# MarvelMathesh/sincformer-metacog-speech-enhancement

Hardware: AMD Instinct MI355X
Metric: audio frames/sec/GPU (16 kHz, 512-frame utts) + mask RMSE vs CPU ref (higher is better)
Workload: dtype fp16 MFMA operands (PerceptionAgent, fusion, Conformer GEMMs, heads) + bf16 attention core, fp32 accumulate (ops.POLICIES['mixed']); 1 GPU; B256 x 512-frame utterances (L40880, T512) forward; batch_per_gpu=256, samples=40880, frames_per_utt=512, launch=eager launches, streams=2, precision_policy=mixed

## Files before the change

### include/sincformer_hip.h

```cpp
#ifndef SINCFORMER_HIP_H
#define SINCFORMER_HIP_H
#ifdef __cplusplus
extern "C" {
#endif

#define SFM_OK 0
#define SFM_ERR_ARG (-1)
#define SFM_ERR_SHAPE (-2)
#define SFM_ERR_LAUNCH (-3)
#define SFM_DT_BF16 0
#define SFM_DT_F16 1

#define SFM_EPI_NONE 0
#define SFM_EPI_SWISH 1
#define SFM_EPI_GELU 2
#define SFM_EPI_RESID 3
#define SFM_EPI_GLU 4
#define SFM_EPI_SIGMOID 5
#define SFM_EPI_TANH_SCALE 6
#define SFM_EPI_SIGMA 7
#define SFM_EPI_CPEA 8

int sfm_abi_version(void);

// ... 145 lines not shown
int sfm_sinc_wgrad(const float* x, const void* dy, int dy_f32, float* dfilt, float* scratch, int B, int L, int C, int K,
                   int dtype, void* stream);
long long sfm_sinc_shift_len(int L);
int sfm_sinc_shift_pack(const float* x, void* xs, int B, int L, int dtype, void* stream);
int sfm_sinc_wgrad16(const void* dy, const void* xs, float* dW, int B, int L, int C, int dtype, float* ws, long long ws_floats,
                     void* stream);
int sfm_gn_bwd_reduce(const void* dout, int dout_f32, const void* x1, int x1_f32, const float* sc1, const float* sh1,
                      const float* mean1, const float* rstd1, const void* x2, int x2_f32, const float* sc2,
                      const float* sh2, const float* mean2, const float* rstd2, float* S, int B, int L, int C, int G,
                      int act, int dtype, float* ws, void* stream);
long long sfm_gn_bwd_reduce_ws_floats(int B, int L, int C);
int sfm_gn_bwd_coefs(float* S, const float* gamma1, const float* rstd1, const float* gamma2, const float* rstd2,
                     float* coef1, float* coef2, float* dparam, int B, int L, int C, int G, void* stream);
int sfm_gn_bwd_apply(const void* dout, int dout_f32, const void* x1, int x1_f32, const float* sc1, const float* sh1,
                     const float* mean1, const float* rstd1, const float* coef1, void* dx1, int dx1_f32, const void* x2,
                     int x2_f32, const float* sc2, const float* sh2, const float* mean2, const float* rstd2,
                     const float* coef2, void* dx2, int dx2_f32, int B, int L, int C, int G, int act, int dtype,
                     void* stream);
int sfm_maa_update_stats(const float* sigma, long long n, double* acc, float* stats, long long* num_updates, float momentum,
                         void* stream);
int sfm_maa_forward(const float* sigma, const float* stats, const float* params, float* logits, float* probs,
                    long long* decisions, float* confidence, long long n, void* stream);
int sfm_maa_backward(const float* sigma, const float* stats, const float* params, const float* g_logits, const float* g_probs,
                     const float* g_conf, float* dsigma, void* H1, void* H2, void* dZ1, void* dZ2, void* GL, void* XN,
                     long long n, int dtype, void* stream);
int sfm_vq_forward(const float* x, const float* centroids, int M, float* q, long long* idx, double* acc, long long n,
                   void* stream);
int sfm_vq_backward(const float* x, const long long* idx, const float* centroids, int M, const float* g_q,
                    const float* g_loss, float beta, float* dx, float* dcent, long long n, void* stream);
int sfm_sumsq(const float* g, long long n, double* out, double* ws, void* stream);
int sfm_adamw_step(float* p, float* g, float* m, float* v, long long n, double* ctl, float lr, float beta1, float beta2,
                   float eps, float wd, float inv_scale, float max_norm, int write_back_grad, void* stream);
int sfm_adamw_step_masked(float* p, float* g, float* m, float* v, long long n, double* ctl, float lr, float beta1, float beta2,
                          float eps, float wd, float inv_scale, float max_norm, int write_back_grad, const long long* spans,
                          const float* touched, int n_params, void* stream);
int sfm_adamw_step_scaled(float* p, float* g, float* m, float* v, long long n, double* ctl, float lr, float beta1, float beta2,
                          float eps, float wd, float inv_world, float max_norm, int write_back_grad, const long long* spans,
                          const float* touched, int n_params, float* loss_scale, float growth_factor, float backoff_factor,
                          int growth_interval, void* stream);
long long sfm_tn_ws_floats(int M, int N, int K);
int sfm_gemm16_tn(const void* G, const void* X, float* dW, float* db, int M, int N, int K, int ldg, int ldx, int ldw,
                  int dtype, float* ws, long long ws_floats, void* stream);
int sfm_conv_wgrad16(const void* G, const void* x, float* dW, float* db, int B, int Lout, int Lin, int Cin, int N, int ksize,
                     int stride, int pad, long long x_batch_stride, int ldg, int ldw, int dtype, float* ws, long long ws_floats,
                     void* stream);
long long sfm_colsum_ws_floats(int M, int N);
int sfm_colsum(const void* G, float* out, int M, int N, int ldg, int g_f32, int dtype, float* ws, void* stream);
long long sfm_layernorm_bwd_ws_floats(int M, int D);
int sfm_layernorm_bwd(const float* x, const float* gamma, const float* dy, const float* dres, float* dx,
                      float* dgamma, float* dbeta, int M, int D, int ldx, int ld, float eps, float* ws, void* stream);
int sfm_layernorm_bwd_ex(const float* x, const float* gamma, const void* dy, int dy_16, const float* dres, float* dx,
                         float* dgamma, float* dbeta, int M, int D, int ldx, int ldy, int ld, float eps, int dtype,
                         float* ws, void* stream);
int sfm_layernorm_bwd_next(const float* x, const float* gamma, const void* dy, int dy_16, const float* dres, float* dx,
                           float* dgamma, float* dbeta, int M, int D, int ldx, int ldy, int ld, float eps, int dtype,
                           void* next16, float next_alpha, float next_p, unsigned int next_seed, float* ws, void* stream);
int sfm_ew_train(const void* z, const void* g, void* out, long long M, int N, int mode, int g_f32, int out_f32,
                 float alpha, float p, unsigned int seed, int dtype, void* stream);
long long sfm_col_stats_ws_floats(int M, int C);
int sfm_col_stats(const float* y, const float* aux, const float* mean, const float* rstd, float* S, int M, int C, float* ws,
                  void* stream);
int sfm_add_cols(const float* a, const float* b, float* out, long long M, int C, int Cb, long long lda, long long ldb, long long ldo,
                 void* stream);
int sfm_lstm_hprev16(const float* h, void* out, int B, int T, int H, int dtype, void* stream);
int sfm_bn_finalize(const float* S, const float* gamma, const float* beta, float* run_mean, float* run_var, float* mean,
                    float* rstd, float* sc, float* sh, int C, long long M, float eps, float momentum, int eval_mode,
                    void* stream);
int sfm_bn_swish_bwd(const void* g, const float* y, const float* mean, const float* rstd, const float* gamma,
                     const float* beta, float* S, float* dy, int M, int C, int g_f32, int pass, int dtype,
                     float* ws, void* stream);
long long sfm_dwconv_wgrad_scratch_floats(int B, int T, int C, int KS);
int sfm_dwconv_wgrad(const void* x, const float* dy, float* dw, float* db, float* scratch, int B, int T, int C, int KS,
                     int dtype, void* stream);
int sfm_attention_fwd_train(const void* qkv, void* out, float* lse, int B, int T, int H, int hd, int ldqkv,
                            int ldo, int koff, int voff, long long qkv_batch_stride, long long o_batch_stride,
                            float scale, float p_drop, unsigned int seed, int dtype, void* stream);
int sfm_attention_bwd(const void* qkv, const void* O, const void* dO, const float* lse, float* delta, void* dqkv,
                      int B, int T, int H, int hd, int ldqkv, int ldo, int koff, int voff, float p_drop,
                      unsigned int seed, int dtype, void* stream);
int sfm_lin256(const void* A, const void* W, const float* bias, void* out, int M, int NW, int lda, int ldo, int glu, int dtype,
               int out_dtype, void* stream);
int sfm_ln_lin256(const float* X32, int ldx, const float* lnw, const float* lnb, float eps, const void* W, const float* bias,
                  void* out, int M, int NW, int ldo, int glu, int dtype, int out_dtype, void* stream);
int sfm_headpool_frames_per_tile(int Tin, int Tout);
int sfm_headpool(const void* xd, const void* W, const float* bias, void* pooled, float* gn_partial, int B, int Tin, int Tout, int NW,
                 int lda, int ldp, int gcols, int dtype, void* stream);

int sfm_bilstm_layer(const float* xg, const float* whh, float* out, int B, int T, int H, int dtype, void* stream);
int sfm_bilstm_layer_ex(const float* xg, const float* whh, float* out, int B, int T, int H, int w16, void* stream);
int sfm_bilstm_layer_train_ex(const float* xg, const float* whh, float* out, float* save, int B, int T, int H, int w16, void* stream);
int sfm_bilstm_layer_train(const float* xg, const float* whh, float* out, float* save, int B, int T, int H, int dtype,
                           void* stream);
int sfm_bilstm_layer_bwd(const float* save, const float* whh, const float* dout, float* dxg, int B, int T, int H,
                         void* stream);
int sfm_memory_fwd(const float* emb, const float* params, float* bias_out, float* gate_out, int* top_idx,
                   float* sim_out, int B, int key_dim, int value_dim, int slots, float temperature, void* stream);
long long sfm_memory_param_floats(int key_dim, int value_dim, int slots);
int sfm_memory_bwd(const float* emb, const float* params, const float* d_out, const float* d_gate, float* d_emb,
                   float* dparams, int B, int key_dim, int value_dim, int slots, float temperature, float* ws, void* stream);

#ifdef __cplusplus
}
#endif
#endif
```

### sincformer_metacog_speech_enhancement_amd/functional.py

```python
import math
import numpy as np
import torch

from . import ops

N_FFT, HOP, WIN = 256, 80, 160
N_FREQ = N_FFT // 2 + 1
SINC_ON_16BIT_MFMA = True
FUSE_LD = 1088


def _f32(t):
    return t.detach().float().contiguous()


def sub(sd, prefix):
    p = prefix + "."
    return {k[len(p):]: v for k, v in sd.items() if k.startswith(p)}


def add_to16(x32, y32, C):
    M = x32.numel() // C
    dev = x32.device
    one = _const(dev, C, 1.0)
# ... 259 lines not shown
        bsh = _f32(sd["batch_norm.bias"]) - _f32(sd["batch_norm.running_mean"]) * bsc + _f32(sd["depthwise.bias"]) * bsc
        folded = (_f32(sd["depthwise.weight"].reshape(D, KS)).t().contiguous(), bsc.contiguous(), bsh.contiguous())
    return {"dw_folded": folded, "ln_w": _f32(sd["layer_norm.weight"]), "ln_b": _f32(sd["layer_norm.bias"]),
            "pw1": ops.pack_linear(sd["pointwise1.weight"].reshape(2 * D, D), sd["pointwise1.bias"], glu=True),
            "dw_w": _f32(sd["depthwise.weight"].reshape(D, -1)), "dw_b": _f32(sd["depthwise.bias"]),
            "bn_w": _f32(sd["batch_norm.weight"]), "bn_b": _f32(sd["batch_norm.bias"]),
            "bn_m": _f32(sd["batch_norm.running_mean"]), "bn_v": _f32(sd["batch_norm.running_var"]),
            "pw2": ops.pack_linear(sd["pointwise2.weight"].reshape(D, D), sd["pointwise2.bias"])}


def pack_block(sd, num_heads=4, index=None):
    with ops.stage("block", index):
        return {"ff1": pack_ffn(sub(sd, "ff1")), "mhsa": pack_mhsa(sub(sd, "mhsa"), num_heads), "conv": pack_convmod(sub(sd, "conv")),
                "ff2": pack_ffn(sub(sd, "ff2")), "fn_w": _f32(sd["final_norm.weight"]), "fn_b": _f32(sd["final_norm.bias"]),
                "index": index}


def _ln16(x32, w, b, act=0):
    out = torch.empty(x32.shape, device=x32.device, dtype=ops.compute_dtype())
    ops.layernorm(x32, w, b, out16=out, act=act)
    return out


def _ffn_fusable(x32, pk):
    return FUSED_FFN and "fused" in pk and x32.is_contiguous()


def ffn_forward_ln(x32, pk, ln_w, ln_b, ln_f32, want_y):
    w1, b1, w2, b2 = pk["fused"]
    return ops.ffn_fused_ln(x32, pk["ln_w"], pk["ln_b"], w1, b1, w2, b2, ln_w, ln_b, ln_f32, want_y=want_y, alpha=0.5)


def ffn_forward(x32, pk):
    if FUSED_FFN and "fused" in pk and x32.is_contiguous():
        w1, b1, w2, b2 = pk["fused"]
        return ops.ffn_fused(x32, pk["ln_w"], pk["ln_b"], w1, b1, w2, b2, alpha=0.5)
    h = _ln16(x32, pk["ln_w"], pk["ln_b"])
    u = ops.linear16(h, pk["w1"], epi=ops.EPI_SWISH)
    return ops.linear16(u, pk["w2"], epi=ops.EPI_RESID, resid=x32, alpha=0.5)


def mhsa_forward(x32, pk, B, T, H, h=None, index=None, seg=None):
    D = x32.shape[1]
    bdt = ops.compute_dtype()
    adt = ops.stage_dtype("attn", index) if D // H == 64 else bdt
    if pk["heads"] != H:
        raise RuntimeError("packed attention weights were scaled for %d heads, got %d" % (pk["heads"], H))
    if h is None:
        qkv = ops.ln_linear16(x32, pk["ln_w"], pk["ln_b"], pk["win"], out_dtype=adt)
    else:
        qkv = ops.linear16(h, pk["win"], out_dtype=adt)
    if seg is not None:
        tb = seg.tables(x32.device, H if D // H == 64 else None)
        args = (qkv, tb["frame_off"], tb["attn_items", H] if D // H == 64 else None, seg.B, seg.max_T, seg.sum_T, H, D // H)
        if adt is bdt:
            o = ops.attention_varlen(*args, prescaled=True, sum_T2=seg.sum_T2)
        else:
            with ops.stage("attn", index):
                o = ops.attention_varlen(*args, prescaled=True, out_dtype=bdt, sum_T2=seg.sum_T2)
    elif adt is bdt:
        o = ops.attention(qkv, B, T, H, D // H, prescaled=True)
    else:
        with ops.stage("attn", index):
            o = ops.attention(qkv, B, T, H, D // H, prescaled=True, out_dtype=bdt)
    return ops.linear16(o, pk["wout"], epi=ops.EPI_RESID, resid=x32, alpha=1.0)


def _dw_folded_any(pk):
    f = pk["dw_folded"] or pk.get("dw_folded_any")
    if f is None:
        bsc = pk["bn_w"] * torch.rsqrt(pk["bn_v"] + 1e-5)
        bsh = pk["bn_b"] - pk["bn_m"] * bsc + pk["dw_b"] * bsc
        f = pk["dw_folded_any"] = (pk["dw_w"].t().contiguous(), bsc.contiguous(), bsh.contiguous())
    return f


def convmod_forward(x32, pk, B, T, seg=None):
    D = x32.shape[1]
    g = ops.ln_linear16(x32, pk["ln_w"], pk["ln_b"], pk["pw1"], epi=ops.EPI_GLU)
    if seg is not None:
        tb = seg.tables(x32.device)
        wT, sc, sh = _dw_folded_any(pk)
        d = ops.dwconv_folded_varlen(g, wT, sc, sh, tb["frame_off"], tb["conv_tiles"], seg.B, seg.max_T, seg.sum_T, D)
    elif pk["dw_folded"] is not None:
        d = ops.dwconv_folded(g, pk["dw_folded"][0], pk["dw_folded"][1], pk["dw_folded"][2], B, T, D)
    else:
        d = ops.dwconv_bn_swish(g, pk["dw_w"], pk["dw_b"], pk["bn_w"], pk["bn_b"], pk["bn_m"], pk["bn_v"], B, T, D)
    return ops.linear16(d, pk["pw2"], epi=ops.EPI_RESID, resid=x32, alpha=1.0)


def block_forward(x32, pk, B, T, H, want16=False, seg=None):
    with ops.stage("block", pk.get("index")):
        return _block_forward(x32, pk, B, T, H, want16, seg)


def _block_forward(x32, pk, B, T, H, want16, seg=None):
    if _ffn_fusable(x32, pk["ff1"]) and x32.shape[1] == 256:
        x, h = ffn_forward_ln(x32, pk["ff1"], pk["mhsa"]["ln_w"], pk["mhsa"]["ln_b"], False, True)
        x = mhsa_forward(x, pk["mhsa"], B, T, H, h=h, index=pk.get("index"), seg=seg)
        x = convmod_forward(x, pk["conv"], B, T, seg=seg)
        if not want16 and _ffn_fusable(x, pk["ff2"]):
            return ffn_forward_ln(x, pk["ff2"], pk["fn_w"], pk["fn_b"], True, False)[1]
        x = ffn_forward(x, pk["ff2"])
    else:
        x = ffn_forward(x32, pk["ff1"])
        x = mhsa_forward(x, pk["mhsa"], B, T, H, index=pk.get("index"), seg=seg)
        x = convmod_forward(x, pk["conv"], B, T, seg=seg)
        x = ffn_forward(x, pk["ff2"])
    out = torch.empty_like(x)
    out16 = torch.empty(x.shape, device=x.device, dtype=ops.compute_dtype()) if want16 else None
    ops.layernorm(x, pk["fn_w"], pk["fn_b"], out16=out16, out32=out)
    return (out, out16) if want16 else out


def pack_complex_conformer(sd, num_blocks, num_heads=4):
    nf2 = sd["input_proj.weight"].shape[1]
    with ops.stage("front"):
        win = ops.pack_linear(sd["input_proj.weight"], sd["input_proj.bias"], k_pad_to=ops.round_up(nf2, 64))
    with ops.stage("tail"):
        wout = ops.pack_linear(sd["output_proj.weight"], sd["output_proj.bias"])
    return {"in": win, "out": wout,
            "blocks": [pack_block(sub(sd, "blocks.%d" % i), num_heads, i) for i in range(num_blocks)], "nf2": nf2}


def complex_conformer_core(x16, pk, B, T, H, out_dtype=None):
    with ops.stage("front"):
        x = ops.linear16(x16, pk["in"], out_dtype=torch.float32)
    skip = x
    for bp in pk["blocks"]:
        x = block_forward(x, bp, B, T, H)
    with ops.stage("tail"):
        y16 = add_to16(x, skip, x.shape[1])
        return ops.linear16(y16, pk["out"], out_dtype=out_dtype or ops.compute_dtype())


def complex_conformer_forward(stft_real, stft_imag, pk, H):
    B, T, nf = stft_real.shape
    M = B * T
    sr, si = stft_real.contiguous(), stft_imag.contiguous()
    ld = pk["in"].Kpad
    with ops.stage("front"):
        x16 = torch.empty(M, ld, device=sr.device, dtype=ops.compute_dtype())
        ops.convert_rows(sr, x16, M, nf, nf, nf, ld)
        ops.convert_rows(si, x16[:, nf:], M, nf, ld - nf, nf, ld)
    y = complex_conformer_core(x16, pk, B, T, H, out_dtype=torch.float32).reshape(B, T, 2 * nf)
    return y[..., :nf], y[..., nf:]


def pack_perception(sd, sample_rate):
    with ops.stage("pa"):
        return _pack_perception(sd, sample_rate)


def _pack_perception(sd, sample_rate):
    pk = {"fs": float(sample_rate)}
    for k in ("low_hz_", "band_hz_", "window", "n_"):
        pk[k] = _f32(sd["sinc_conv." + k]).reshape(-1)
    pk["K"] = pk["window"].numel()
    pk["C0"] = pk["low_hz_"].numel()
    pk["sn_w"], pk["sn_b"] = _f32(sd["sinc_norm.weight"]), _f32(sd["sinc_norm.bias"])
    pk["blocks"] = []
    for i in range(3):
        s = sub(sd, "conv_blocks.%d" % i)
        cout = s["main.0.weight"].shape[0]
        pk["blocks"].append({
            "c1": ops.pack_linear(s["main.0.weight"], s["main.0.bias"]), "g1w": _f32(s["main.1.weight"]), "g1b": _f32(s["main.1.bias"]),
# ... 350 lines not shown
```

### sincformer_metacog_speech_enhancement_amd/lib.py

```python
import ctypes
import os

import torch

_HERE = os.path.dirname(os.path.abspath(__file__))
LIB_PATH = os.environ.get("SFM_LIB_PATH") or os.path.join(_HERE, "libsincformer_hip.so")

c_vp = ctypes.c_void_p
c_i = ctypes.c_int
c_ll = ctypes.c_longlong
c_f = ctypes.c_float

SIGNATURES = {
    "sfm_abi_version": [],
    "sfm_gemm16": [c_vp, c_vp, c_vp, c_vp, c_vp, c_vp, c_i, c_i, c_i, c_i, c_i, c_i, c_i, c_i, c_ll, c_i, c_i, c_i,
                   c_i, c_ll, c_i, c_ll, c_f, c_i, c_i, c_i, c_i, c_i, c_vp],
    "sfm_gemm16_ex": [c_vp, c_vp, c_vp, c_vp, c_vp, c_vp, c_i, c_i, c_i, c_i, c_i, c_i, c_i, c_i, c_ll, c_i, c_i, c_i,
                   c_i, c_ll, c_i, c_ll, c_f, c_i, c_i, c_i, c_i, c_i, c_i, c_vp],
    "sfm_gemm16_train": [c_vp, c_vp, c_vp, c_vp, c_vp, c_vp, c_i, c_i, c_i, c_i, c_i, c_i, c_i, c_i, c_ll, c_i, c_i, c_i,
                   c_i, c_ll, c_i, c_ll, c_f, c_i, c_i, c_i, c_i, c_i, c_i, c_f, ctypes.c_uint, c_vp],
    "sfm_conv16p": [c_vp, c_vp, c_vp, c_vp, c_vp, c_vp, c_vp, c_vp, c_vp, c_vp, c_vp, c_vp, c_vp, c_vp, c_i, c_i, c_i, c_i, c_i,
                    c_i, c_i, c_i, c_i, c_i, c_vp],
    "sfm_framed_gemm_f32": [c_vp, c_vp, c_vp, c_vp, c_vp, c_vp, c_i, c_i, c_i, c_ll, c_i, c_i, c_i, c_i, c_i, c_i,
                            c_i, c_ll, c_ll, c_ll, c_i, c_i, c_i, c_i, c_vp],
# ... 14 lines not shown
    "sfm_pool_time_affine": [c_vp, c_vp, c_vp, c_vp, c_vp, c_i, c_i, c_i, c_i, c_ll, c_ll, c_i, c_vp],
    "sfm_pool_time_affine16": [c_vp, c_i, c_vp, c_vp, c_vp, c_vp, c_i, c_i, c_i, c_i, c_ll, c_ll, c_i, c_vp],
    "sfm_stft_lognorm_pack": [c_vp, c_vp, c_vp, c_ll, c_i, c_i, c_ll, c_i, c_vp],
    "sfm_stft_lognorm_bwd": [c_vp, c_vp, c_vp, c_vp, c_vp, c_ll, c_i, c_ll, c_vp],
    "sfm_polar_mask": [c_vp, c_vp, c_vp, c_vp, c_vp, c_vp, c_vp, c_vp, c_vp, c_vp, c_i, c_ll, c_i, c_f, c_ll, c_ll,
                       c_vp],
    "sfm_complex_mul": [c_vp, c_vp, c_vp, c_vp, c_vp, c_vp, c_ll, c_vp],
    "sfm_istft_ola": [c_vp, c_vp, c_vp, c_i, c_i, c_i, c_i, c_i, c_i, c_ll, c_vp],
    "sfm_pack_spec": [c_vp, c_vp, c_vp, c_ll, c_i, c_i, c_ll, c_vp],
    "sfm_sinc_filters": [c_vp, c_vp, c_vp, c_vp, c_vp, c_vp, c_i, c_i, c_i, c_f, c_f, c_f, c_vp],
    "sfm_ffn_fused": [c_vp, c_vp, c_vp, c_vp, c_vp, c_vp, c_vp, c_vp, c_i, c_i, c_i, c_f, c_f, c_i, c_vp],
    "sfm_ffn_fused_ln": [c_vp, c_vp, c_vp, c_vp, c_vp, c_vp, c_vp, c_vp, c_i, c_i, c_i, c_f, c_f, c_vp, c_vp, c_vp, c_i, c_i,
                         c_vp],
    "sfm_sinc_fir16_tiles": [c_i],
    "sfm_sinc_fir16": [c_vp, c_vp, c_vp, c_vp, c_vp, c_i, c_i, c_i, c_i, c_i, c_i, c_vp],
    "sfm_sinc_fir16_ex": [c_vp, c_vp, c_vp, c_vp, c_vp, c_i, c_i, c_i, c_i, c_i, c_i, c_i, c_vp],
    "sfm_framed_gemm_split16": [c_vp, c_vp, c_vp, c_vp, c_vp, c_i, c_i, c_i, c_ll, c_i, c_i, c_i, c_i, c_i, c_i, c_i, c_i, c_ll,
                                c_ll, c_i, c_vp],
    "sfm_wave_moments": [c_vp, c_vp, c_vp, c_i, c_i, c_vp, c_vp],
    "sfm_spec_sums": [c_vp, c_vp, c_vp, c_vp, c_vp, c_ll, c_vp, c_vp],
    "sfm_enhancer_loss_finalize": [c_vp, c_vp, c_vp, c_vp, c_i, c_i, c_ll, c_i, c_vp, c_vp],
    "sfm_sisnr_bwd": [c_vp, c_vp, c_vp, c_vp, c_i, c_i, c_f, c_vp],
    "sfm_spec_loss_bwd": [c_vp, c_vp, c_vp, c_vp, c_vp, c_vp, c_vp, c_ll, c_i, c_ll, c_i, c_i, c_f, c_vp],
    "sfm_stft_adjoint_ola": [c_vp, c_vp, c_vp, c_i, c_i, c_i, c_i, c_i, c_i, c_i, c_vp],
    "sfm_polar_mask_bwd": [c_vp, c_vp, c_vp, c_vp, c_vp, c_vp, c_vp, c_vp, c_ll, c_ll, c_i, c_f, c_ll, c_ll, c_vp],
    "sfm_attention_bwd_generic": [c_vp, c_vp, c_vp, c_vp, c_vp, c_vp, c_i, c_i, c_i, c_i, c_i, c_i, c_i, c_i, c_f, ctypes.c_uint, c_i,
                                  c_vp],
    "sfm_ssnr_frames": [c_vp, c_vp, c_vp, c_i, c_i, c_i, c_i, c_f, c_f, c_vp],
    "sfm_stoi_frames": [c_vp, c_vp, c_vp, c_vp, c_vp, c_vp, c_vp, c_i, c_i, c_i, c_vp],
    "sfm_lsd_frames": [c_vp, c_vp, c_vp, c_vp, c_vp, c_i, c_i, c_i, c_vp],
    "sfm_ssnr_frames_varlen": [c_vp, c_vp, c_vp, c_vp, c_vp, c_i, c_i, c_i, c_i, c_f, c_f, c_vp],
    "sfm_stoi_frames_varlen": [c_vp, c_vp, c_vp, c_vp, c_vp, c_vp, c_vp, c_vp, c_i, c_i, c_i, c_vp],
    "sfm_lsd_frames_varlen": [c_vp, c_vp, c_vp, c_vp, c_vp, c_vp, c_i, c_i, c_i, c_vp],
    "sfm_wave_moments_varlen": [c_vp, c_vp, c_vp, c_vp, c_i, c_i, c_vp],
    "sfm_sinc_wgrad_scratch_floats": [c_i, c_i, c_i, c_i],
    "sfm_sinc_wgrad": [c_vp, c_vp, c_i, c_vp, c_vp, c_i, c_i, c_i, c_i, c_i, c_vp],
    "sfm_sinc_shift_len": [c_i],
    "sfm_sinc_shift_pack": [c_vp, c_vp, c_i, c_i, c_i, c_vp],
    "sfm_sinc_wgrad16": [c_vp, c_vp, c_vp, c_i, c_i, c_i, c_i, c_vp, c_ll, c_vp],
    "sfm_gemm16_swish": [c_vp, c_vp, c_vp, c_vp, c_vp, c_vp, c_i, c_i, c_i, c_i, c_i, c_i, c_i, c_i, c_f, ctypes.c_uint, c_i, c_vp],
    "sfm_gn_bwd_reduce": [c_vp, c_i, c_vp, c_i, c_vp, c_vp, c_vp, c_vp, c_vp, c_i, c_vp, c_vp, c_vp, c_vp, c_vp, c_i, c_i, c_i,
                          c_i, c_i, c_i, c_vp, c_vp],
    "sfm_gn_bwd_coefs": [c_vp, c_vp, c_vp, c_vp, c_vp, c_vp, c_vp, c_vp, c_i, c_i, c_i, c_i, c_vp],
    "sfm_gn_bwd_apply": [c_vp, c_i, c_vp, c_i, c_vp, c_vp, c_vp, c_vp, c_vp, c_vp, c_i, c_vp, c_i, c_vp, c_vp, c_vp, c_vp,
                         c_vp, c_vp, c_i, c_i, c_i, c_i, c_i, c_i, c_i, c_vp],
    "sfm_maa_update_stats": [c_vp, c_ll, c_vp, c_vp, c_vp, c_f, c_vp],
    "sfm_maa_forward": [c_vp, c_vp, c_vp, c_vp, c_vp, c_vp, c_vp, c_ll, c_vp],
    "sfm_maa_backward": [c_vp, c_vp, c_vp, c_vp, c_vp, c_vp, c_vp, c_vp, c_vp, c_vp, c_vp, c_vp, c_vp, c_ll, c_i, c_vp],
    "sfm_vq_forward": [c_vp, c_vp, c_i, c_vp, c_vp, c_vp, c_ll, c_vp],
    "sfm_vq_backward": [c_vp, c_vp, c_vp, c_i, c_vp, c_vp, c_f, c_vp, c_vp, c_ll, c_vp],
    "sfm_sumsq": [c_vp, c_ll, c_vp, c_vp, c_vp],
    "sfm_adamw_step": [c_vp, c_vp, c_vp, c_vp, c_ll, c_vp, c_f, c_f, c_f, c_f, c_f, c_f, c_f, c_i, c_vp],
    "sfm_adamw_step_masked": [c_vp, c_vp, c_vp, c_vp, c_ll, c_vp, c_f, c_f, c_f, c_f, c_f, c_f, c_f, c_i, c_vp, c_vp, c_i, c_vp],
    "sfm_adamw_step_scaled": [c_vp, c_vp, c_vp, c_vp, c_ll, c_vp, c_f, c_f, c_f, c_f, c_f, c_f, c_f, c_i, c_vp, c_vp, c_i, c_vp,
                              c_f, c_f, c_i, c_vp],
    "sfm_tn_ws_floats": [c_i, c_i, c_i],
    "sfm_colsum_ws_floats": [c_i, c_i],
    "sfm_layernorm_bwd_ws_floats": [c_i, c_i],
    "sfm_col_stats_ws_floats": [c_i, c_i],
    "sfm_gn_bwd_reduce_ws_floats": [c_i, c_i, c_i],
    "sfm_gemm16_tn": [c_vp, c_vp, c_vp, c_vp, c_i, c_i, c_i, c_i, c_i, c_i, c_i, c_vp, c_ll, c_vp],
    "sfm_conv_wgrad16": [c_vp, c_vp, c_vp, c_vp, c_i, c_i, c_i, c_i, c_i, c_i, c_i, c_i, c_ll, c_i, c_i, c_i, c_vp, c_ll, c_vp],
    "sfm_colsum": [c_vp, c_vp, c_i, c_i, c_i, c_i, c_i, c_vp, c_vp],
    "sfm_layernorm_bwd": [c_vp, c_vp, c_vp, c_vp, c_vp, c_vp, c_vp, c_i, c_i, c_i, c_i, c_f, c_vp, c_vp],
    "sfm_layernorm_bwd_ex": [c_vp, c_vp, c_vp, c_i, c_vp, c_vp, c_vp, c_vp, c_i, c_i, c_i, c_i, c_i, c_f, c_i, c_vp, c_vp],
    "sfm_layernorm_bwd_next": [c_vp, c_vp, c_vp, c_i, c_vp, c_vp, c_vp, c_vp, c_i, c_i, c_i, c_i, c_i, c_f, c_i, c_vp, c_f, c_f,
                               ctypes.c_uint, c_vp, c_vp],
    "sfm_ew_train": [c_vp, c_vp, c_vp, c_ll, c_i, c_i, c_i, c_i, c_f, c_f, ctypes.c_uint, c_i, c_vp],
    "sfm_col_stats": [c_vp, c_vp, c_vp, c_vp, c_vp, c_i, c_i, c_vp, c_vp],
    "sfm_add_cols": [c_vp, c_vp, c_vp, c_ll, c_i, c_i, c_ll, c_ll, c_ll, c_vp],
    "sfm_lstm_hprev16": [c_vp, c_vp, c_i, c_i, c_i, c_i, c_vp],
    "sfm_bn_finalize": [c_vp, c_vp, c_vp, c_vp, c_vp, c_vp, c_vp, c_vp, c_vp, c_i, c_ll, c_f, c_f, c_i, c_vp],
    "sfm_bn_swish_bwd": [c_vp, c_vp, c_vp, c_vp, c_vp, c_vp, c_vp, c_vp, c_i, c_i, c_i, c_i, c_i, c_vp, c_vp],
    "sfm_dwconv_wgrad": [c_vp, c_vp, c_vp, c_vp, c_vp, c_i, c_i, c_i, c_i, c_i, c_vp],
    "sfm_dwconv_wgrad_scratch_floats": [c_i, c_i, c_i, c_i],
    "sfm_attention_fwd_train": [c_vp, c_vp, c_vp, c_i, c_i, c_i, c_i, c_i, c_i, c_i, c_i, c_ll, c_ll, c_f, c_f,
                                ctypes.c_uint, c_i, c_vp],
    "sfm_attention_bwd": [c_vp, c_vp, c_vp, c_vp, c_vp, c_vp, c_i, c_i, c_i, c_i, c_i, c_i, c_i, c_i, c_f,
                          ctypes.c_uint, c_i, c_vp],
    "sfm_lin256": [c_vp, c_vp, c_vp, c_vp, c_i, c_i, c_i, c_i, c_i, c_i, c_i, c_vp],
    "sfm_headpool_frames_per_tile": [c_i, c_i],
    "sfm_headpool": [c_vp, c_vp, c_vp, c_vp, c_vp, c_i, c_i, c_i, c_i, c_i, c_i, c_i, c_i, c_vp],
    "sfm_ln_lin256": [c_vp, c_i, c_vp, c_vp, c_f, c_vp, c_vp, c_vp, c_i, c_i, c_i, c_i, c_i, c_i, c_vp],
    "sfm_bilstm_layer": [c_vp, c_vp, c_vp, c_i, c_i, c_i, c_i, c_vp],
    "sfm_bilstm_layer_ex": [c_vp, c_vp, c_vp, c_i, c_i, c_i, c_i, c_vp],
    "sfm_bilstm_layer_train": [c_vp, c_vp, c_vp, c_vp, c_i, c_i, c_i, c_i, c_vp],
    "sfm_bilstm_layer_train_ex": [c_vp, c_vp, c_vp, c_vp, c_i, c_i, c_i, c_i, c_vp],
    "sfm_bilstm_layer_bwd": [c_vp, c_vp, c_vp, c_vp, c_i, c_i, c_i, c_vp],
    "sfm_memory_fwd": [c_vp, c_vp, c_vp, c_vp, c_vp, c_vp, c_i, c_i, c_i, c_i, c_f, c_vp],
    "sfm_memory_bwd": [c_vp, c_vp, c_vp, c_vp, c_vp, c_vp, c_i, c_i, c_i, c_i, c_f, c_vp, c_vp],
    "sfm_memory_param_floats": [c_i, c_i, c_i],
    "sfm_framed_gemm_f32_varlen": [c_vp, c_vp, c_vp, c_vp, c_vp, c_vp, c_i, c_i, c_i, c_i, c_i, c_i, c_i, c_i, c_i, c_ll, c_ll,
                                   c_i, c_i, c_i, c_vp],
    "sfm_framed_gemm_split16_varlen": [c_vp, c_vp, c_vp, c_vp, c_vp, c_vp, c_vp, c_i, c_i, c_i, c_i, c_i, c_i, c_i, c_i, c_i, c_i,
                                       c_ll, c_i, c_vp],
    "sfm_attention_fwd_varlen": [c_vp, c_vp, c_vp, c_vp, c_i, c_i, c_i, c_i, c_i, c_i, c_i, c_i, c_i, c_i, c_f, c_i, c_i, c_vp],
    "sfm_dwconv_folded_varlen": [c_vp, c_vp, c_vp, c_vp, c_vp, c_vp, c_vp, c_i, c_i, c_i, c_i, c_i, c_i, c_i, c_i, c_i, c_vp],
    "sfm_istft_ola_varlen": [c_vp, c_vp, c_vp, c_vp, c_vp, c_i, c_i, c_i, c_i, c_i, c_ll, c_vp],
}

_lib = None


class HipExtensionMissing(RuntimeError):
    pass


def load():
    global _lib
    if _lib is not None:
        return _lib
    if not os.path.exists(LIB_PATH):
        raise HipExtensionMissing(
            "libsincformer_hip.so not built (%s). Run `python -m sincformer_metacog_speech_enhancement_amd.build` "
            "or __graft_entry__.build(); there is no CPU fallback." % LIB_PATH)
    lib = ctypes.CDLL(LIB_PATH)
    for name, args in SIGNATURES.items():
        try:
            fn = getattr(lib, name)
        except AttributeError as e:
            raise HipExtensionMissing("symbol %s missing from %s" % (name, LIB_PATH)) from e
        fn.argtypes = args
        fn.restype = c_ll if name.endswith("_scratch_floats") or name.endswith("_ws_floats") or name in ("sfm_sinc_shift_len", "sfm_memory_param_floats") else c_i
    _lib = lib
    return lib


_ERR = {-1: "bad argument", -2: "unsupported shape", -3: "kernel launch failed"}


def check(rc, name):
    if rc != 0:
        raise RuntimeError("%s failed: %s (%d)" % (name, _ERR.get(rc, "error"), rc))
```

### sincformer_metacog_speech_enhancement_amd/ops.py

```python
import ctypes
import math
import numpy as np
import torch

from . import lib as _lib

EPI_NONE, EPI_SWISH, EPI_GELU, EPI_RESID, EPI_GLU, EPI_SIGMOID, EPI_TANH_SCALE, EPI_SIGMA, EPI_CPEA = range(9)

_DT_ID = {torch.bfloat16: 0, torch.float16: 1}
import os as _os
TRAIN_DTYPE = torch.float16
_state = {"dtype": TRAIN_DTYPE, "gemm_variant": int(_os.environ.get("SFM_GEMM_VARIANT", "0"))}


def set_gemm_variant(v):
    _state["gemm_variant"] = int(v)



_DT_NAMES = {"bf16": torch.bfloat16, "bfloat16": torch.bfloat16, "f16": torch.float16, "fp16": torch.float16,
             "float16": torch.float16}
STAGES = ("pa", "front", "block", "attn", "tail")
POLICIES = {
    "bf16": {s: torch.bfloat16 for s in STAGES},
# ... 295 lines not shown
    lda = cin if lda is None else lda
    out_f32 = 1 if out.dtype == torch.float32 else (0 if out.dtype == _state["dtype"] else 2)
    if A.dtype != _state["dtype"] or pw.w.dtype != _state["dtype"]:
        raise RuntimeError("gemm16: operand formats %s / %s do not match the stage's %s (precision policy)" %
                           (A.dtype, pw.w.dtype, _state["dtype"]))
    if p_drop > 0.0:
        _call("gemm16", L.sfm_gemm16_train, (_p(A), _p(pw.w), _p(pw.bias), _p(out), _p(resid), _p(gn_partial), B, Lout, Lin, cin,
                                             lda, pw.ksize, stride, pad, a_batch_stride, pw.Kpad, pw.N, pw.Npad, ldo,
                                             o_batch_stride, ldr, r_batch_stride, float(alpha), epi, out_f32, gn_group, nsplit,
                                             _dt(), _state["gemm_variant"], float(p_drop), int(seed) & 0xffffffff, _stream()),
              *_cost_of("gemm16", locals()))
        return out
    _call("gemm16", L.sfm_gemm16_ex, (_p(A), _p(pw.w), _p(pw.bias), _p(out), _p(resid), _p(gn_partial), B, Lout, Lin, cin, lda,
                      pw.ksize, stride, pad, a_batch_stride, pw.Kpad, pw.N, pw.Npad, ldo, o_batch_stride, ldr, r_batch_stride,
                      float(alpha), epi, out_f32, gn_group, nsplit, _dt(), _state["gemm_variant"], _stream()),
          *_cost_of("gemm16", locals()))
    return out


def conv16p_supported(cin, n, ksize, stride, pad, two_inputs, skip):
    if cin % 64:
        return False
    key = (ksize, stride, pad, n)
    if skip:
        return key == (7, 2, 3, 128)
    return (key == (7, 2, 3, 256) and two_inputs) or (key in ((3, 1, 1, 128), (3, 1, 1, 256)) and not two_inputs) or \
        (key in ((5, 2, 2, 256), (1, 2, 0, 256)) and two_inputs)


def conv16p(x1, sc1, sh1, pw, out, *, B, Lin, stride, pad, x2=None, sc2=None, sh2=None, gn_partial=None, gn_group=0,
            skip_pw=None, out_s=None, gn_partial_s=None):
    _need_dev(x1, out)
    L = _lib.load()
    cin, N, ks = pw.cin, pw.N, pw.ksize
    dt = _state["dtype"]
    if x1.dtype != dt or pw.w.dtype != dt or (x2 is not None and x2.dtype != dt):
        raise RuntimeError("conv16p: operand formats do not match the stage's %s (precision policy)" % dt)
    if pw.Npad != N or pw.Kpad != ks * cin or (skip_pw is not None and (skip_pw.Npad != N or skip_pw.Kpad != cin)):
        raise RuntimeError("conv16p: weights must be packed without padding")
    out_f32 = 1 if out.dtype == torch.float32 else (0 if out.dtype == dt else 2)
    Lout = (Lin + 2 * pad - ks) // stride + 1
    nin = 2 if x2 is not None else 1
    flops = 2.0 * B * Lout * N * (ks * cin + (cin if skip_pw is not None else 0))
    nbytes = B * Lin * cin * 2.0 * nin + B * Lout * N * out.element_size() * (2 if skip_pw is not None else 1) + N * ks * cin * 2.0
    _call("conv16p", L.sfm_conv16p, (_p(x1), _p(sc1), _p(sh1), _p(x2), _p(sc2), _p(sh2), _p(pw.w), _p(pw.bias), _p(out),
                                     _p(gn_partial), _p(skip_pw.w if skip_pw is not None else None),
                                     _p(skip_pw.bias if skip_pw is not None else None), _p(out_s), _p(gn_partial_s), B, Lin, cin, N,
                                     ks, stride, pad, out_f32, gn_group, _dt(), _stream()),
          flops, nbytes, tag="Lout%d Cin%d N%d k%d s%d in%d%s" % (B * Lout, cin, N, ks, stride, nin, " +skip" if skip_pw is not None else ""))
    return out


_LIN256 = {"on": _os.environ.get("SFM_LIN256", "1") != "0"}


def set_lin256(flag):
    _LIN256["on"] = bool(flag)


def _lin256_ok(x16, pw, epi, out, resid, nsplit, p_drop):
    return (_LIN256["on"] and _state["gemm_variant"] == 0 and epi in (EPI_NONE, EPI_GLU) and (epi == EPI_GLU) == bool(pw.glu) and
            pw.K == 256 and pw.Kpad == 256 and pw.ksize == 1 and pw.Npad % (128 if pw.glu else 64) == 0 and
            (pw.Npad == (2 * pw.N if pw.glu else pw.N)) and pw.Npad <= 2048 and
            resid is None and nsplit == 0 and p_drop == 0.0 and
            (out.dtype in (torch.float16, torch.bfloat16) or (out.dtype == torch.float32 and not pw.glu and out.stride(0) % 4 == 0)) and
            x16.shape[0] >= 4096 and x16.stride(1) == 1 and out.stride(1) == 1 and x16.stride(0) % 8 == 0 and
            (out.stride(0) % 8 == 0 or out.dtype == torch.float32) and
            x16.dtype == _state["dtype"] and pw.w.dtype == _state["dtype"])


def lin256(x16, pw, out):
    _need_dev(x16, out)
    L = _lib.load()
    M, ld = x16.shape[0], x16.stride(0)
    odt_id = 2 if out.dtype == torch.float32 else (1 if out.dtype == torch.float16 else 0)
    osz = 4.0 if out.dtype == torch.float32 else 2.0
    _call("gemm16", L.sfm_lin256, (_p(x16), _p(pw.w), _p(pw.bias), _p(out), M, pw.Npad, ld, out.stride(0), 1 if pw.glu else 0,
                                   _dt(), odt_id, _stream()),
          2.0 * M * pw.Npad * 256, M * 256 * 2.0 + pw.Npad * 512.0 + M * pw.N * osz,
          tag="M%d N%d K256 lin256%s o%d" % (M, pw.Npad, " glu" if pw.glu else "", int(osz)))
    return out


_HEADPOOL = {"on": _os.environ.get("SFM_HEADPOOL", "1") != "0"}


def set_headpool(flag):
    _HEADPOOL["on"] = bool(flag)


def headpool_tiles(Tin, Tout):
    if not _HEADPOOL["on"] or _state["gemm_variant"] != 0:
        return None
    fpt = int(_lib.load().sfm_headpool_frames_per_tile(int(Tin), int(Tout)))
    return (fpt, (Tout + fpt - 1) // fpt) if fpt > 0 else None


def headpool(xd16, pw, pooled16, part, B, Tin, Tout, gcols=16):
    _need_dev(xd16, pooled16, part)
    L = _lib.load()
    if xd16.dtype != _state["dtype"] or pw.w.dtype != _state["dtype"] or pooled16.dtype != _state["dtype"]:
        raise RuntimeError("headpool: operands must be in the stage's format")
    _call("gemm16", L.sfm_headpool, (_p(xd16), _p(pw.w), _p(pw.bias), _p(pooled16), _p(part), B, Tin, Tout, pw.Npad, xd16.stride(1),
                                     pooled16.stride(1), gcols, _dt(), _stream()),
          2.0 * B * Tin * pw.Npad * 256, B * Tin * 512.0 + pw.Npad * 512.0 + B * Tout * pw.Npad * 2.0,
          tag="M%d N%d K256 headpool->T%d" % (B * Tin, pw.Npad, Tout))


def ln_linear16(x32, ln_w, ln_b, pw, epi=EPI_NONE, out_dtype=None, eps=1e-5):
    M = x32.shape[0]
    out = torch.empty(M, pw.N, device=x32.device, dtype=out_dtype or _state["dtype"])
    fused = (_LIN256["on"] and _state["gemm_variant"] == 0 and epi in (EPI_NONE, EPI_GLU) and (epi == EPI_GLU) == bool(pw.glu) and
             pw.K == 256 and pw.Kpad == 256 and pw.ksize == 1 and pw.Npad % (128 if pw.glu else 64) == 0 and
             pw.Npad == (2 * pw.N if pw.glu else pw.N) and pw.Npad <= 2048 and out.dtype in (torch.float16, torch.bfloat16) and
             M >= 4096 and x32.dtype == torch.float32 and x32.stride(1) == 1 and x32.stride(0) % 4 == 0 and
             x32.data_ptr() % 16 == 0 and ln_w.numel() == 256 and pw.w.dtype == _state["dtype"])
    if fused:
        _need_dev(x32, out)
        L = _lib.load()
        lw, lb = ln_w.detach().float().contiguous(), ln_b.detach().float().contiguous()
        _call("gemm16", L.sfm_ln_lin256, (_p(x32), x32.stride(0), _p(lw), _p(lb), float(eps), _p(pw.w), _p(pw.bias), _p(out), M, pw.Npad,
                                          out.stride(0), 1 if pw.glu else 0, _dt(), 1 if out.dtype == torch.float16 else 0, _stream()),
              2.0 * M * pw.Npad * 256, M * 256 * 4.0 + pw.Npad * 512.0 + M * pw.N * 2.0,
              tag="M%d N%d K256 ln+lin256%s" % (M, pw.Npad, " glu" if pw.glu else ""))
        return out
    h16 = torch.empty(M, ln_w.numel(), device=x32.device, dtype=_state["dtype"])
    layernorm(x32, ln_w, ln_b, out16=h16, eps=eps)
    return linear16(h16, pw, epi=epi, out=out)


def linear16(x16, pw, epi=EPI_NONE, out_dtype=None, resid=None, alpha=1.0, out=None, nsplit=0, p_drop=0.0, seed=0):
    M, ld = x16.shape[0], x16.stride(0)
    if out is None:
        odt = out_dtype or (torch.float32 if epi == EPI_RESID else _state["dtype"])
        out = torch.empty(M, pw.N, device=x16.device, dtype=odt)
    if _lin256_ok(x16, pw, epi, out, resid, nsplit, p_drop):
        return lin256(x16, pw, out)
    gemm16(x16, pw, out, B=1, Lout=M, Lin=M, a_batch_stride=0, lda=ld, ldo=out.stride(0), o_batch_stride=0, epi=epi,
           resid=resid, ldr=(resid.stride(0) if resid is not None else 0), alpha=alpha, nsplit=nsplit, p_drop=p_drop,
           seed=seed)
    return out


def linear16_swish(x16, pw, p_drop=0.0, seed=0, aux=None):
    L = _lib.load()
    M, ld = x16.shape[0], x16.stride(0)
    dt = _state["dtype"]
    out = torch.empty(M, pw.N, device=x16.device, dtype=dt)
    out2 = torch.empty(M, pw.N, device=x16.device, dtype=dt) if aux is None else None
    _call("gemm16", L.sfm_gemm16_swish, (_p(x16), _p(pw.w), _p(pw.bias), _p(out), _p(aux), _p(out2), M, pw.cin, ld, pw.Kpad, pw.N,
                                         pw.Npad, pw.N, 0 if aux is None else 1, float(p_drop), int(seed) & 0xffffffff, _dt(),
                                         _stream()), 2.0 * M * pw.N * pw.K, M * (pw.cin + 2.0 * pw.N) * 2.0 + pw.Npad * pw.Kpad * 2.0,
          tag="M%d N%d K%d swish%s" % (M, pw.N, pw.K, "" if aux is None else "_bwd"))
    return (out2, out) if aux is None else out


def framed_gemm(sig, Wt, out, *, B, M, Ls, sig_batch_stride, hop, padl, K, N, o_batch_stride, ldm, ldn, mode=0,
                bias=None, out2=None, nsplit=0, gn_partial=None, gn_group=0):
    _need_dev(sig, Wt, out)
    L = _lib.load()
    Kpad, Npad = Wt.shape
    out_f32 = 1 if out.dtype == torch.float32 else 0
    _call("framed_gemm_f32", L.sfm_framed_gemm_f32, (_p(sig), _p(Wt), _p(bias), _p(out), _p(out2), _p(gn_partial), B, M, Ls,
                               sig_batch_stride, hop, padl, K, Kpad, N, Npad, nsplit, o_batch_stride, ldm, ldn, mode,
                               out_f32, gn_group, _dt(), _stream()),
          *_cost_of("framed_gemm_f32", locals()))
# ... 964 lines not shown
```

Baseline: 8.478 million STFT frames/s (whole job).

## Fuse depthwise conv, BN-swish and pointwise linear with residual into one kernel

Adds a HIP kernel that computes the 31-tap depthwise conv with folded BN and swish into LDS, then runs the 256x256 pointwise projection with MFMA and adds the fp32 residual, all in one launch. The conv-module forward uses it by default when the shapes and dtype fit. This removes the round trip of the intermediate fp16 activation through global memory and one kernel launch. In exchange it brings a large LDS footprint (about 160 KB, which limits occupancy), a hand-tuned triple-buffered weight pipeline, and dwconv weights rounded to fp16 in the fdot2 path, which may change numerics slightly.

```diff
diff --git a/include/sincformer_hip.h b/include/sincformer_hip.h
--- a/include/sincformer_hip.h
+++ b/include/sincformer_hip.h
@@ -251,6 +251,9 @@
                int out_dtype, void* stream);
 int sfm_ln_lin256(const float* X32, int ldx, const float* lnw, const float* lnb, float eps, const void* W, const float* bias,
                   void* out, int M, int NW, int ldo, int glu, int dtype, int out_dtype, void* stream);
+int sfm_dwconv_lin256_resid(const void* g, const float* wT, const float* sc, const float* sh, const void* W, const float* bias,
+                            const float* resid, float* out, int B, int T, int ldg, int ldr, int ldo, float alpha, int dtype,
+                            void* stream);
 int sfm_headpool_frames_per_tile(int Tin, int Tout);
 int sfm_headpool(const void* xd, const void* W, const float* bias, void* pooled, float* gn_partial, int B, int Tin, int Tout, int NW,
                  int lda, int ldp, int gcols, int dtype, void* stream);
diff --git a/sincformer_metacog_speech_enhancement_amd/csrc/block_fuse.hip b/sincformer_metacog_speech_enhancement_amd/csrc/block_fuse.hip
--- /dev/null
+++ b/sincformer_metacog_speech_enhancement_amd/csrc/block_fuse.hip
@@ -0,0 +1,260 @@
+#include "sfm_common.h"
+
+#define BF_BM 128
+#define BF_C 256
+#define BF_KS 31
+#define BF_STAGE 32768
+#define BF_IMG 16384
+#define BF_IMG_OFF (3 * BF_STAGE)
+#define BF_PATCH_OFF 65536
+#define BF_PATCH_ROWS 160
+#define BF_BIAS_OFF (BF_PATCH_OFF + BF_PATCH_ROWS * 512)
+#define BF_LDS (BF_BIAS_OFF + BF_C * 4)
+
+typedef __attribute__((address_space(3))) void* bf_lds_ptr_t;
+typedef _Float16 bf_h2 __attribute__((ext_vector_type(2)));
+typedef __amdgpu_buffer_rsrc_t bf_rsrc_t;
+
+template <int N>
+__device__ __forceinline__ void bf_wait_vmcnt() {
+  asm volatile("s_waitcnt vmcnt(%0)" ::"n"(N) : "memory");
+}
+__device__ __forceinline__ void bf_frag_read(u32x4& dst, uint32_t lds_addr) {
+  asm volatile("ds_read_b128 %0, %1" : "=v"(dst) : "v"(lds_addr) : "memory");
+}
+template <int N>
+__device__ __forceinline__ void bf_frag_wait(u32x4& frag) {
+  asm volatile("s_waitcnt lgkmcnt(%1)" : "+v"(frag) : "n"(N) : "memory");
+}
+__device__ __forceinline__ void bf_barrier() {
+  asm volatile("s_waitcnt lgkmcnt(0)" ::: "memory");
+  __builtin_amdgcn_s_barrier();
+  asm volatile("" ::: "memory");
+}
+
+struct BfRows {
+  int mbase, nvalid, ldr, ldo, r_bytes, o_bytes;
+  float alpha;
+};
+
+__device__ __forceinline__ void bf_resid_load(bf_rsrc_t r_rs, const BfRows& R, int cc, int tid, f32x4 (&r)[4]) {
+#pragma unroll
+  for (int i = 0; i < 2; ++i)
+#pragma unroll
+    for (int j = 0; j < 2; ++j) {
+      const int idx = tid + 512 * j;
+      const int row = idx >> 3, pc = idx & 7;
+      const int lc = pc ^ ((row >> 1) & 7);
+      const int n = cc * 64 + i * 32 + lc * 4;
+      const int voff = (row < R.nvalid) ? ((R.mbase + row) * R.ldr + n) * 4 : R.r_bytes;
+      r[i * 2 + j] = __builtin_bit_cast(f32x4, __builtin_amdgcn_raw_buffer_load_b128(r_rs, voff, 0, 0));
+    }
+}
+
+__device__ __forceinline__ void bf_lin256_resid(unsigned char* smem, const u32x4 (&hf)[16], bf_rsrc_t w_rs, bf_rsrc_t r_rs,
+                                                bf_rsrc_t o_rs, const float* bs, const BfRows& R, f32x4 (&rs0)[4], f32x4 (&rs1)[4],
+                                                int tid, int wave, int l31, int hl) {
+  unsigned char* img0 = smem + BF_IMG_OFF;
+  const int r1 = (wave >> 1) * 32 + l31;
+  auto w_piece = [&](int cc, int stage, int i) {
+    const int inst = wave * 4 + i;
+    const int row = inst * 2 + hl;
+    const int lc = l31 ^ (row & 15);
+    const int voff = ((cc * 64 + row) * BF_C + lc * 8) * 2;
+    __builtin_amdgcn_raw_ptr_buffer_load_lds(w_rs, (bf_lds_ptr_t)(smem + stage * BF_STAGE + inst * 1024), 16, voff, 0, 0, 0);
+  };
+#pragma unroll
+  for (int cc = 0; cc < 3; ++cc)
+#pragma unroll
+    for (int i = 0; i < 4; ++i) w_piece(cc, cc, i);
+
+  const int half = wave & 1;
+  const int n1 = half * 32 + l31;
+  const uint32_t w_lane = (uint32_t)(uintptr_t)(bf_lds_ptr_t)smem + (uint32_t)(n1 * 512);
+  const int hx4 = (hl ^ (n1 & 15)) << 4;
+  auto epi_quad = [&](const f32x16& s, int cc, int q) {
+    const f32x4 bv = *reinterpret_cast<const f32x4*>(bs + cc * 64 + half * 32 + 8 * q + 4 * hl);
+    float y[4];
+#pragma unroll
+    for (int e = 0; e < 4; ++e) y[e] = s[4 * q + e] + bv[e];
+    unsigned char* img = img0 + (half ? BF_IMG : 0);
+    const int ch = 2 * q + hl;
+    *reinterpret_cast<f32x4*>(img + r1 * 128 + ((ch ^ ((r1 >> 1) & 7)) << 4)) = f32x4{y[0], y[1], y[2], y[3]};
+  };
+  auto store_chunk = [&](int cc, const f32x4 (&r)[4]) {
+#pragma unroll
+    for (int i = 0; i < 2; ++i)
+#pragma unroll
+      for (int j = 0; j < 2; ++j) {
+        const int idx = tid + 512 * j;
+        const int row = idx >> 3, pc = idx & 7;
+        const int lc = pc ^ ((row >> 1) & 7);
+        const f32x4 v = *reinterpret_cast<const f32x4*>(img0 + (i ? BF_IMG : 0) + row * 128 + pc * 16);
+        const f32x4 rv = r[i * 2 + j];
+        const f32x4 y = {rv[0] + R.alpha * v[0], rv[1] + R.alpha * v[1], rv[2] + R.alpha * v[2], rv[3] + R.alpha * v[3]};
+        const int n = cc * 64 + i * 32 + lc * 4;
+        const int voff = (row < R.nvalid) ? ((R.mbase + row) * R.ldo + n) * 4 : R.o_bytes;
+        __builtin_amdgcn_raw_buffer_store_b128(__builtin_bit_cast(u32x4, y), o_rs, voff, 0, 0);
+      }
+  };
+  auto mfma_chunk = [&](int cc, f32x16& sn, const f32x16& sp, bool with_epi, bool with_refill) {
+#pragma unroll
+    for (int r = 0; r < 16; ++r) sn[r] = 0.f;
+    const uint32_t fbase = w_lane + (uint32_t)((cc % 3) * BF_STAGE);
+    u32x4 fw[4];
+#pragma unroll
+    for (int k = 0; k < 4; ++k) bf_frag_read(fw[k], fbase + (uint32_t)(hx4 ^ (k << 5)));
+#pragma unroll
+    for (int k = 0; k < 16; ++k) {
+      if (k <= 12) bf_frag_wait<3>(fw[k & 3]);
+      else if (k == 13) bf_frag_wait<2>(fw[k & 3]);
+      else if (k == 14) bf_frag_wait<1>(fw[k & 3]);
+      else bf_frag_wait<0>(fw[k & 3]);
+      sn = F16::mfma(fw[k & 3], hf[k], sn);
+      if (k + 4 < 16) bf_frag_read(fw[k & 3], fbase + (uint32_t)(hx4 ^ ((k + 4) << 5)));
+      if (with_epi && (k & 3) == 1) epi_quad(sp, cc - 1, k >> 2);
+      if (with_refill && (k & 3) == 3) w_piece(cc + 2, (cc + 2) % 3, k >> 2);
+    }
+  };
+
+  f32x16 sa, sb;
+  bf_wait_vmcnt<8>();
+  bf_barrier();
+  mfma_chunk(0, sa, sa, false, false);
+  bf_wait_vmcnt<4>();
+  bf_barrier();
+  mfma_chunk(1, sb, sa, true, true);
+  bf_wait_vmcnt<4>();
+  bf_barrier();
+  store_chunk(0, rs0);
+  bf_barrier();
+  bf_resid_load(r_rs, R, 2, tid, rs0);
+  mfma_chunk(2, sa, sb, true, false);
+  bf_wait_vmcnt<8>();
+  bf_barrier();
+  store_chunk(1, rs1);
+  bf_barrier();
+  bf_resid_load(r_rs, R, 3, tid, rs1);
+  mfma_chunk(3, sb, sa, true, false);
+  bf_barrier();
+  store_chunk(2, rs0);
+  bf_barrier();
+#pragma unroll
+  for (int q = 0; q < 4; ++q) epi_quad(sb, 3, q);
+  bf_barrier();
+  store_chunk(3, rs1);
+}
+
+__global__ __launch_bounds__(512) void dwconv_lin256_resid_kernel(const u16* __restrict__ g, const float* __restrict__ wT,
+                                                                  const float* __restrict__ sc, const float* __restrict__ sh,
+                                                                  const u16* __restrict__ W, const float* __restrict__ bias,
+                                                                  const float* __restrict__ resid, float* __restrict__ out, int T,
+                                                                  int ldg, int ldr, int ldo, int g_bytes, int r_bytes, int o_bytes,
+                                                                  float alpha) {
+  extern __shared__ __attribute__((aligned(16))) unsigned char smem[];
+  const u16* xs = reinterpret_cast<const u16*>(smem + BF_PATCH_OFF);
+  float* bs = reinterpret_cast<float*>(smem + BF_BIAS_OFF);
+  constexpr int padl = (BF_KS - 1) / 2;
+  constexpr int NP = (BF_KS + 1) / 2;
+  constexpr int NR = BF_KS + 3;
+  constexpr int w_bytes = BF_C * BF_C * 2;
+
+  const int tid = threadIdx.x, lane = tid & 63;
+  const int wave = __builtin_amdgcn_readfirstlane(tid >> 6);
+  const int l31 = lane & 31, hl = lane >> 5;
+  const int t0 = blockIdx.x * BF_BM;
+  const long long row0 = (long long)blockIdx.y * T;
+  const BfRows R = {(int)row0 + t0, T - t0, ldr, ldo, r_bytes, o_bytes, alpha};
+  auto g_rs = __builtin_amdgcn_make_buffer_rsrc((void*)(g + row0 * ldg), 0, g_bytes, 0x00020000);
+  auto w_rs = __builtin_amdgcn_make_buffer_rsrc((void*)W, 0, w_bytes, 0x00020000);
+  auto r_rs = __builtin_amdgcn_make_buffer_rsrc((void*)resid, 0, r_bytes, 0x00020000);
+  auto o_rs = __builtin_amdgcn_make_buffer_rsrc((void*)out, 0, o_bytes, 0x00020000);
+
+#pragma unroll
+  for (int i = 0; i < BF_PATCH_ROWS / 16; ++i) {
+    const int inst = wave * (BF_PATCH_ROWS / 16) + i;
+    const int row = inst * 2 + hl;
+    const int t = t0 - padl + row;
+    const int voff = (t >= 0 && t < T) ? (t * ldg + l31 * 8) * 2 : g_bytes;
+    __builtin_amdgcn_raw_ptr_buffer_load_lds(g_rs, (bf_lds_ptr_t)(smem + BF_PATCH_OFF + inst * 1024), 16, voff, 0, 0, 0);
+  }
+  const int p = tid & 127, grp = tid >> 7;
+  const int c = 2 * p;
+  bf_h2 w0[NP], w1[NP];
+#pragma unroll
+  for (int j = 0; j < NP; ++j) {
+    const f32x2 a = *reinterpret_cast<const f32x2*>(wT + (2 * j) * BF_C + c);
+    f32x2 bq = {0.f, 0.f};
+    if (2 * j + 1 < BF_KS) bq = *reinterpret_cast<const f32x2*>(wT + (2 * j + 1) * BF_C + c);
+    w0[j] = bf_h2{(_Float16)a[0], (_Float16)bq[0]};
+    w1[j] = bf_h2{(_Float16)a[1], (_Float16)bq[1]};
+  }
+  const float s0 = sc[c], s1 = sc[c + 1], h0 = sh[c], h1 = sh[c + 1];
+  if (tid < BF_C) bs[tid] = bias ? bias[tid] : 0.f;
+  bf_wait_vmcnt<0>();
+  __syncthreads();
+  f32x4 rs0[4], rs1[4];
+  bf_resid_load(r_rs, R, 0, tid, rs0);
+  bf_resid_load(r_rs, R, 1, tid, rs1);
+
+  for (int tl = grp * 32; tl < (grp + 1) * 32; tl += 4) {
+    uint32_t d[NR + 1];
+#pragma unroll
+    for (int k = 0; k < NR; ++k) d[k] = *reinterpret_cast<const uint32_t*>(&xs[(tl + k) * BF_C + c]);
+    d[NR] = d[NR - 1];
+    float a0[4] = {0.f, 0.f, 0.f, 0.f}, a1[4] = {0.f, 0.f, 0.f, 0.f};
+#pragma unroll
+    for (int o = 0; o < 4; ++o) {
+#pragma unroll
+      for (int j = 0; j < NP; ++j) {
+        const uint32_t lo = __builtin_amdgcn_perm(d[o + 2 * j + 1], d[o + 2 * j], 0x05040100u);
+        const uint32_t hi = __builtin_amdgcn_perm(d[o + 2 * j + 1], d[o + 2 * j], 0x07060302u);
+        a0[o] = __builtin_amdgcn_fdot2(w0[j], __builtin_bit_cast(bf_h2, lo), a0[o], false);
+        a1[o] = __builtin_amdgcn_fdot2(w1[j], __builtin_bit_cast(bf_h2, hi), a1[o], false);
+      }
+    }
+#pragma unroll
+    for (int o = 0; o < 4; ++o) {
+      const int r = tl + o;
+      float y0 = a0[o] * s0 + h0, y1 = a1[o] * s1 + h1;
+      y0 = swish_f(y0);
+      y1 = swish_f(y1);
+      *reinterpret_cast<uint32_t*>(smem + r * 512 + (((p >> 2) ^ (r & 15)) << 4) + (p & 3) * 4) = pack2<F16>(y0, y1);
+    }
+  }
+  __syncthreads();
+  const int r1 = (wave >> 1) * 32 + l31;
+  u32x4 hf[16];
+#pragma unroll
+  for (int s = 0; s < 16; ++s) hf[s] = *reinterpret_cast<const u32x4*>(smem + r1 * 512 + (((2 * s + hl) ^ (r1 & 15)) << 4));
+  __syncthreads();
+  bf_lin256_resid(smem, hf, w_rs, r_rs, o_rs, bs, R, rs0, rs1, tid, wave, l31, hl);
+}
+
+extern "C" int sfm_dwconv_lin256_resid(const void* g, const float* wT, const float* sc, const float* sh, const void* W,
+                                       const float* bias, const float* resid, float* out, int B, int T, int ldg, int ldr, int ldo,
+                                       float alpha, int dtype, void* stream) {
+  if (!g || !wT || !sc || !sh || !W || !resid || !out) return SFM_ERR_ARG;
+  if (dtype != SFM_DT_F16) return SFM_ERR_ARG;
+  if (B <= 0 || T <= 0 || B > 65535 || ldg < BF_C || (ldg % 8) != 0 || ldr < BF_C || (ldr % 4) != 0 || ldo < BF_C || (ldo % 4) != 0)
+    return SFM_ERR_SHAPE;
+  if ((((uintptr_t)g | (uintptr_t)W | (uintptr_t)resid | (uintptr_t)out) % 16) != 0 || (((uintptr_t)wT | (uintptr_t)sc | (uintptr_t)sh) % 8) != 0)
+    return SFM_ERR_SHAPE;
+  const long long M = (long long)B * T;
+  const long long g_bytes = ((long long)(T - 1) * ldg + BF_C) * 2;
+  const long long r_bytes = ((M - 1) * ldr + BF_C) * 4, o_bytes = ((M - 1) * ldo + BF_C) * 4;
+  if (g_bytes >= (1LL << 31) || r_bytes >= (1LL << 31) || o_bytes >= (1LL << 31)) return SFM_ERR_SHAPE;
+  hipStream_t st = (hipStream_t)stream;
+  int dev = 0;
+  if (hipGetDevice(&dev) != hipSuccess || dev < 0 || dev >= 64) return SFM_ERR_LAUNCH;
+  static bool attr_set[64] = {false};
+  if (!attr_set[dev]) {
+    if (hipFuncSetAttribute((const void*)dwconv_lin256_resid_kernel, hipFuncAttributeMaxDynamicSharedMemorySize, 160 * 1024) != hipSuccess)
+      return SFM_ERR_LAUNCH;
+    attr_set[dev] = true;
+  }
+  const dim3 grid((T + BF_BM - 1) / BF_BM, B), block(512);
+  SFM_LAUNCH(dwconv_lin256_resid_kernel, grid, block, BF_LDS, st, (const u16*)g, wT, sc, sh, (const u16*)W, bias, resid, out, T, ldg,
+             ldr, ldo, (int)g_bytes, (int)r_bytes, (int)o_bytes, alpha);
+  return SFM_OK;
+}
diff --git a/sincformer_metacog_speech_enhancement_amd/functional.py b/sincformer_metacog_speech_enhancement_amd/functional.py
--- a/sincformer_metacog_speech_enhancement_amd/functional.py
+++ b/sincformer_metacog_speech_enhancement_amd/functional.py
@@ -365,6 +365,8 @@
         tb = seg.tables(x32.device)
         wT, sc, sh = _dw_folded_any(pk)
         d = ops.dwconv_folded_varlen(g, wT, sc, sh, tb["frame_off"], tb["conv_tiles"], seg.B, seg.max_T, seg.sum_T, D)
+    elif ops._block_fuse_conv_ok(g, pk["dw_folded"], pk["pw2"], x32, B, T):
+        return ops.dwconv_lin256_resid(g, pk["dw_folded"][0], pk["dw_folded"][1], pk["dw_folded"][2], pk["pw2"], x32, B, T, alpha=1.0)
     elif pk["dw_folded"] is not None:
         d = ops.dwconv_folded(g, pk["dw_folded"][0], pk["dw_folded"][1], pk["dw_folded"][2], B, T, D)
     else:
diff --git a/sincformer_metacog_speech_enhancement_amd/lib.py b/sincformer_metacog_speech_enhancement_amd/lib.py
--- a/sincformer_metacog_speech_enhancement_amd/lib.py
+++ b/sincformer_metacog_speech_enhancement_amd/lib.py
@@ -120,6 +120,7 @@
     "sfm_headpool_frames_per_tile": [c_i, c_i],
     "sfm_headpool": [c_vp, c_vp, c_vp, c_vp, c_vp, c_i, c_i, c_i, c_i, c_i, c_i, c_i, c_i, c_vp],
     "sfm_ln_lin256": [c_vp, c_i, c_vp, c_vp, c_f, c_vp, c_vp, c_vp, c_i, c_i, c_i, c_i, c_i, c_i, c_vp],
+    "sfm_dwconv_lin256_resid": [c_vp, c_vp, c_vp, c_vp, c_vp, c_vp, c_vp, c_vp, c_i, c_i, c_i, c_i, c_i, c_f, c_i, c_vp],
     "sfm_bilstm_layer": [c_vp, c_vp, c_vp, c_i, c_i, c_i, c_i, c_vp],
     "sfm_bilstm_layer_ex": [c_vp, c_vp, c_vp, c_i, c_i, c_i, c_i, c_vp],
     "sfm_bilstm_layer_train": [c_vp, c_vp, c_vp, c_vp, c_i, c_i, c_i, c_i, c_vp],
diff --git a/sincformer_metacog_speech_enhancement_amd/ops.py b/sincformer_metacog_speech_enhancement_amd/ops.py
--- a/sincformer_metacog_speech_enhancement_amd/ops.py
+++ b/sincformer_metacog_speech_enhancement_amd/ops.py
@@ -401,6 +401,42 @@
     return out
 
 
+def _block_fuse_default():
+    return _os.environ.get("SFM_BLOCK_FUSE", "1") != "0"
+
+
+_BLOCK_FUSE = {"on": _block_fuse_default()}
+
+
+def set_block_fuse(flag):
+    _BLOCK_FUSE["on"] = bool(flag)
+
+
+def _block_fuse_conv_ok(g16, folded, pw, resid, B, T, seg=None, p_drop=0.0):
+    return (_BLOCK_FUSE["on"] and _state["gemm_variant"] == 0 and seg is None and p_drop == 0.0 and folded is not None and
+            _os.environ.get("SFM_DWCONV_DOT", "1") != "0" and
+            _state["dtype"] == torch.float16 and g16.dtype == torch.float16 and pw.w.dtype == torch.float16 and
+            tuple(folded[0].shape) == (31, 256) and folded[0].is_contiguous() and
+            not pw.glu and pw.ksize == 1 and pw.K == 256 and pw.Kpad == 256 and pw.N == 256 and pw.Npad == 256 and
+            g16.dim() == 2 and g16.shape[0] == B * T and g16.shape[1] == 256 and B * T >= 4096 and 0 < B <= 65535 and
+            g16.stride(1) == 1 and g16.stride(0) % 8 == 0 and
+            resid is not None and resid.dtype == torch.float32 and tuple(resid.shape) == (B * T, 256) and
+            resid.stride(1) == 1 and resid.stride(0) % 4 == 0 and
+            B * T * max(resid.stride(0), 256) * 4 < 2 ** 31 and T * g16.stride(0) * 2 < 2 ** 31)
+
+
+def dwconv_lin256_resid(g16, wT, sc, sh, pw, resid, B, T, alpha=1.0):
+    out = torch.empty(B * T, 256, device=g16.device, dtype=torch.float32)
+    _need_dev(g16, out)
+    L = _lib.load()
+    M = B * T
+    _call("gemm16", L.sfm_dwconv_lin256_resid, (_p(g16), _p(wT), _p(sc), _p(sh), _p(pw.w), _p(pw.bias), _p(resid), _p(out), B, T,
+                                                g16.stride(0), resid.stride(0), out.stride(0), float(alpha), _dt(), _stream()),
+          2.0 * M * 256 * 31 + 2.0 * M * 256 * 256, M * 256 * 2.0 + 256 * 512.0 + M * 256 * 8.0,
+          tag="M%d N256 K256 dwconv31+lin256 resid" % M)
+    return out
+
+
 _HEADPOOL = {"on": _os.environ.get("SFM_HEADPOOL", "1") != "0"}
 
 
```

New measurement: 8.525 million STFT frames/s (whole job), median of 3. No clear change (+0.6%).
